# letao1991/EAD-GAN

Measured on AMD Instinct MI355X. Metric: imgs/sec per G+D+E train step, CelebA 64x64 bs=128, higher is better.
Workload: dtype bf16; 1 GPU; EAD-GAN CelebA 64x64x3 full train iteration (G adv + D + info/affine, 3 Adams), batch 128/GPU, hipGraph replay, data-parallel x1; per_gpu_batch=128, global_batch=128, parallelism=dp1

## Files before the change

ead-gan_amd/csrc/igemm_tn8.hip:

```cpp
#include <string.h>
#include <algorithm>

#include "eg_common.h"
#include "igemm_nt.h"

__device__ __forceinline__ int tn8_fsw(int row) { return (row & 3) | (((row >> 3) & 1) << 2); }

__device__ __forceinline__ void tn8_wait(int n) {
    switch (n) {
        case 0: __builtin_amdgcn_s_waitcnt(0 | (7 << 4)); break;
        case 1: __builtin_amdgcn_s_waitcnt(1 | (7 << 4)); break;
        case 2: __builtin_amdgcn_s_waitcnt(2 | (7 << 4)); break;
        case 3: __builtin_amdgcn_s_waitcnt(3 | (7 << 4)); break;
        case 4: __builtin_amdgcn_s_waitcnt(4 | (7 << 4)); break;
        case 5: __builtin_amdgcn_s_waitcnt(5 | (7 << 4)); break;
        case 6: __builtin_amdgcn_s_waitcnt(6 | (7 << 4)); break;
        default: __builtin_amdgcn_s_waitcnt(7 | (7 << 4)); break;
    }
}

template <typename T, int CH>
__global__ __launch_bounds__(512) void igemm_tn8_kernel(const Tn8Params p) {
    constexpr int ROWB = CH * 2;
    constexpr int RPP = 1024 / ROWB;
    constexpr int CPR = ROWB / 16;
    constexpr int NBLK = ROWB / 32;
    constexpr int NI = CH / 32, NJ = CH / 16;
    constexpr int NPP_P = (64 / RPP + 7) / 8;
    constexpr int PW_P = 64 / RPP < 8 ? 64 / RPP : 8;
    constexpr int STAGE_P = 64 * ROWB, STAGE_X = EG_TN8_XSLOTS * ROWB, STAGE = STAGE_P + STAGE_X;
    extern __shared__ __attribute__((aligned(16))) char smem[];
    const int tid = threadIdx.x, lane = tid & 63;
    const int wave = __builtin_amdgcn_readfirstlane(tid >> 6);
    const int tp = wave >> 1, nh = wave & 1;
    const int ay = tp >> 1, ax = tp & 1;
    const int tn_i = blockIdx.x / p.ntc, tc_i = blockIdx.x - tn_i * p.ntc;
    const int n0 = tn_i * CH, c0 = tc_i * CH;
    const int ry = blockIdx.y >> 1, rx = blockIdx.y & 1;
    const int mbeg = blockIdx.z * p.rows_per_split;
    const int mend = min(p.M, mbeg + p.rows_per_split);
    const int nk = (mend - mbeg) >> 6;
    const int OWm = (1 << p.lOW) - 1, OHm = (1 << p.lOH) - 1;
    const unsigned row_bytes = (unsigned)p.C * 2u;
    const int g = lane >> 4, li = lane & 15, q = li >> 2, pc = li & 3;

    int prow[4], xrow[4];
#pragma unroll
    for (int i = 0; i < 4; ++i) {
        const int r = (i >> 1) * 32 + 8 * g + (i & 1) * 4 + q;
        prow[i] = r * ROWB + (tn8_fsw(r) & (NBLK - 1));
        int img, oy;
        if (p.nimg == 1) { img = 0; oy = r >> p.lOW; }
        else { img = r >> (p.lOH + p.lOW); oy = (r >> p.lOW) & OHm; }
        const int px = (img * p.PH + oy + ay) * p.PW + (r & OWm) + ax;
        xrow[i] = px * ROWB + (tn8_fsw(px) & (NBLK - 1));
    }
    auto frag_addr = [&](int rowkey, int blk) { return (rowkey & ~7) + (((blk ^ (rowkey & 7)) << 5) | (pc << 3)); };

    const int c16 = lane % CPR, rsub = lane / CPR;
    const u32x4_t srdP = eg_make_srd(p.P, (unsigned)((size_t)p.M * p.N * 2));
    const u32x4_t srdX = eg_make_srd(p.src, (unsigned)((size_t)p.B * p.H * p.W * p.C * 2));
    unsigned vP[NPP_P];
#pragma unroll
    for (int j = 0; j < NPP_P; ++j) {
        const int r = RPP * (wave + 8 * j) + rsub;
        const int src16 = (((c16 >> 1) ^ (tn8_fsw(r) & (NBLK - 1))) << 1) | (c16 & 1);
        vP[j] = (unsigned)r * (unsigned)p.N * 2u + (unsigned)n0 * 2u + (unsigned)src16 * 16u;
    }
    int xa[5], xdy[5];
#pragma unroll
    for (int j = 0; j < 5; ++j) {
        const unsigned ps = (unsigned)(RPP * (wave + 8 * j) + rsub);
        const unsigned img = (ps * p.inv_plane) >> 20;
        const unsigned rem = ps - img * (unsigned)(p.PH * p.PW);
        const unsigned qy = (rem * p.inv_pw) >> 20, qx = rem - qy * (unsigned)p.PW;
        const int ix = (int)qx * 2 + rx - 1;
        const int src16 = (((c16 >> 1) ^ (tn8_fsw((int)ps) & (NBLK - 1))) << 1) | (c16 & 1);
        const bool ok = (int)ps < p.npix && ix >= 0 && ix < p.W;
        xdy[j] = (int)qy * 2 + ry - 1;
        xa[j] = ok ? (int)(((img * (unsigned)(p.H * p.W) + (unsigned)ix) * row_bytes) + (unsigned)c0 * 2u + (unsigned)src16 * 16u) : -1;
    }
    const unsigned lds0 = (unsigned)(size_t)(__attribute__((address_space(3))) char*)smem + (unsigned)wave * 1024u;

    auto issue = [&](int s, int stage) {
        const int m0s = mbeg + (s << 6);
        const unsigned base = __builtin_amdgcn_readfirstlane(lds0 + (unsigned)stage * STAGE);
        const unsigned soffP = (unsigned)m0s * (unsigned)p.N * 2u;
        if (PW_P == 8 || wave < PW_P) eg_bufdma1f<0>(srdP, vP[0], soffP, base);
        if constexpr (NPP_P > 1) eg_bufdma1f<0x2000>(srdP, vP[NPP_P - 1], soffP, base);
        const int b_s = m0s >> (p.lOH + p.lOW);
        const int oy_s = p.nimg == 1 ? ((m0s >> p.lOW) & OHm) : 0;
        const int ybase = oy_s * 2;
        const int pixbase = (b_s * p.H + ybase) * p.W;
#pragma unroll
        for (int j = 0; j < 5; ++j) {
            if (j < p.npp && (wave + 8 * j) * RPP < p.npix) {
                const int iy = ybase + xdy[j];
                const bool ok = xa[j] >= 0 && iy >= 0 && iy < p.H;
                const unsigned v = ok ? (unsigned)(xa[j] + (pixbase + xdy[j] * p.W) * (int)row_bytes) : EG_OOB;
                if (j == 0) eg_bufdma1f<STAGE_P>(srdX, v, 0u, base);
                if (j == 1) eg_bufdma1f<STAGE_P + 0x2000>(srdX, v, 0u, base);
                if (j == 2) eg_bufdma1f<STAGE_P + 0x4000>(srdX, v, 0u, base);
                if (j == 3) eg_bufdma1f<STAGE_P + 0x6000>(srdX, v, 0u, base);
                if (j == 4) eg_bufdma1f<STAGE_P + 0x8000>(srdX, v, 0u, base);
            }
        }
    };

    f32x4 acc[NI][NJ];
#pragma unroll
    for (int i = 0; i < NI; ++i)
#pragma unroll
        for (int j = 0; j < NJ; ++j) acc[i][j] = (f32x4){0.f, 0.f, 0.f, 0.f};

    typedef __attribute__((address_space(3))) s16x4* lds_s16x4;
    auto tr2 = [&](const char* base, int a_lo, int a_hi) {
        const s16x4 lo = __builtin_amdgcn_ds_read_tr16_b64_v4i16((lds_s16x4)(base + a_lo));
        const s16x4 hi = __builtin_amdgcn_ds_read_tr16_b64_v4i16((lds_s16x4)(base + a_hi));
        return make_uint4(((uint32_t)(uint16_t)lo[0]) | ((uint32_t)(uint16_t)lo[1] << 16), ((uint32_t)(uint16_t)lo[2]) | ((uint32_t)(uint16_t)lo[3] << 16),
                          ((uint32_t)(uint16_t)hi[0]) | ((uint32_t)(uint16_t)hi[1] << 16), ((uint32_t)(uint16_t)hi[2]) | ((uint32_t)(uint16_t)hi[3] << 16));
    };
    auto compute = [&](int stage) {
        const char* sp = smem + stage * STAGE;
        const char* sx = sp + STAGE_P;
#pragma unroll
        for (int kb = 0; kb < 2; ++kb) {
            uint4 af[NI], bfr[NJ];
#pragma unroll
            for (int i = 0; i < NI; ++i) af[i] = tr2(sp, frag_addr(prow[2 * kb], nh * NI + i), frag_addr(prow[2 * kb + 1], nh * NI + i));
#pragma unroll
            for (int j = 0; j < NJ; ++j) bfr[j] = tr2(sx, frag_addr(xrow[2 * kb], j), frag_addr(xrow[2 * kb + 1], j));
#pragma unroll
            for (int i = 0; i < NI; ++i)
#pragma unroll
                for (int j = 0; j < NJ; ++j) {
                    if constexpr (std::is_same<T, f16_t>::value)
                        acc[i][j] = __builtin_amdgcn_mfma_f32_16x16x32_f16(__builtin_bit_cast(f16x8_t, af[i]), __builtin_bit_cast(f16x8_t, bfr[j]), acc[i][j], 0, 0, 0);
                    else
                        acc[i][j] = __builtin_amdgcn_mfma_f32_16x16x32_bf16(__builtin_bit_cast(bf16x8_t, af[i]), __builtin_bit_cast(bf16x8_t, bfr[j]), acc[i][j], 0, 0, 0);
                }
        }
    };
    auto barrier = [&]() {
        __builtin_amdgcn_s_barrier();
        __builtin_amdgcn_sched_barrier(0);
    };

    int per = (PW_P == 8 || wave < PW_P) ? NPP_P : 0;
    for (int j = 0; j < p.npp; ++j) per += (wave + 8 * j) * RPP < p.npix;
    if (nk > 0) issue(0, 0);
    if (nk > 1) issue(1, 1);
    tn8_wait(nk > 1 ? per : 0);
    barrier();
    int st = 0;
    for (int t = 0; t < nk; ++t) {
        const int st2 = st == 0 ? 2 : st - 1;
        const bool more = t + 2 < nk;
        if (more) issue(t + 2, st2);
        compute(st);
        tn8_wait(more ? per : 0);
        barrier();
        st = st == 2 ? 0 : st + 1;
    }

    const int tap = (ry + 2 * ay) * 4 + (rx + 2 * ax);
    float* slab = p.slab + (size_t)blockIdx.z * p.N * 16 * p.C;
#pragma unroll
    for (int i = 0; i < NI; ++i)
#pragma unroll
        for (int r = 0; r < 4; ++r) {
            const int n = n0 + (nh * NI + i) * 16 + g * 4 + r;
            float* row = slab + ((size_t)n * 16 + tap) * p.C + c0 + li;
#pragma unroll
            for (int j = 0; j < NJ; ++j) row[j * 16] = acc[i][j][r];
        }
}

bool eg_tn8_plan(const eg_conv* c, int dtype, Tn8Params& p, int* nsplit, int wgs_target) {
    if (dtype == EG_F32 || c->k != 4 || c->stride != 2 || c->pad != 1 || c->up != 0) return false;
    const int ch = ((c->Cin % 128) == 0 && (c->Cout % 128) == 0) ? 128 : (((c->Cin % 64) == 0 && (c->Cout % 64) == 0) ? 64
                   : (((c->Cin % 32) == 0 && (c->Cout % 32) == 0) ? 32 : 0));
    if (ch == 0 || (c->H & 1) || (c->W & 1)) return false;
    const int OH = c->H / 2, OW = c->W / 2;
    const int lOH = ilog2_exact(OH), lOW = ilog2_exact(OW);
    const long long M = (long long)c->B * OH * OW;
    if (lOH < 0 || lOW < 0 || OW > 64 || (M % 64) != 0) return false;
    if ((size_t)c->B * c->H * c->W * c->Cin * 2 >= 0x7fffffffull || (size_t)M * c->Cout * 2 >= 0x7fffffffull) return false;
    memset(&p, 0, sizeof(p));
    p.B = c->B; p.H = c->H; p.W = c->W; p.C = c->Cin; p.N = c->Cout;
    p.lOH = lOH; p.lOW = lOW; p.M = (int)M;
    if (OH * OW >= 64) { p.nimg = 1; p.OHt = 64 / OW; }
    else { p.nimg = 64 / (OH * OW); p.OHt = OH; }
    p.PH = p.OHt + 1; p.PW = OW + 1;
    p.npix = p.nimg * p.PH * p.PW;
    p.ch = ch;
    const int rpp = 1024 / (ch * 2);
    if ((p.npix + rpp - 1) / rpp * rpp > EG_TN8_XSLOTS) return false;
    p.npp = ((p.npix + rpp - 1) / rpp + 7) / 8;
    if (p.npp > 5) return false;
    p.inv_pw = (1u << 20) / (unsigned)p.PW + 1;
    p.inv_plane = (1u << 20) / (unsigned)(p.PH * p.PW) + 1;
    for (unsigned x = 0; x < 512; ++x)
        if (((x * p.inv_pw) >> 20) != x / (unsigned)p.PW || ((x * p.inv_plane) >> 20) != x / (unsigned)(p.PH * p.PW)) return false;
    p.ntn = c->Cout / ch; p.ntc = c->Cin / ch;
    const long long base = (long long)p.ntn * p.ntc * 4;
    const int target = wgs_target > 0 ? wgs_target : 256;
    long long want = base >= target ? 1 : (target + base - 1) / base;
    const long long steps = M / 64;
    want = std::min(want, std::max(1LL, steps / 4));
    const long long sps = (steps + want - 1) / want;
    p.rows_per_split = (int)(sps * 64);
    *nsplit = (int)((steps + sps - 1) / sps);
    return true;
}

template <typename T, int CH>
static void launch_tn8_ch(const Tn8Params& p, int nsplit, hipStream_t st) {
    constexpr size_t lds = 3 * (size_t)(64 + EG_TN8_XSLOTS) * CH * 2;
    static bool attr_set = false;
    if (!attr_set) {
        (void)hipFuncSetAttribute(reinterpret_cast<const void*>(&igemm_tn8_kernel<T, CH>), hipFuncAttributeMaxDynamicSharedMemorySize, (int)lds);
        attr_set = true;
    }
    hipLaunchKernelGGL((igemm_tn8_kernel<T, CH>), dim3(p.ntn * p.ntc, 4, nsplit), dim3(512), lds, st, p);
}

template <typename T>
void eg_launch_tn8(const Tn8Params& p, int nsplit, hipStream_t st) {
    if (p.ch == 32) launch_tn8_ch<T, 32>(p, nsplit, st);
    else if (p.ch == 64) launch_tn8_ch<T, 64>(p, nsplit, st);
    else launch_tn8_ch<T, 128>(p, nsplit, st);
}
template void eg_launch_tn8<bf16_t>(const Tn8Params&, int, hipStream_t);
template void eg_launch_tn8<f16_t>(const Tn8Params&, int, hipStream_t);
```

Measured before the change: 30750 imgs/s.

## Software-pipeline LDS fragment reads with MFMA and interleave DMA issue in tn8 igemm

Restructures the main loop of the stride-2 4x4 weight-gradient implicit GEMM so fragments for the next k-half are read from LDS while MFMAs run on the current ones. DMA issue for stage t+3 is split into pieces spread across the MFMA loop, with one barrier per iteration placed between the halves. The prologue fills all three stages, and precomputed swizzled LDS addresses replace the per-access frag_addr math. It also simplifies the out-of-bounds checks and adds static asserts, at the cost of higher register pressure and fragile hand-placed waitcnt and barrier ordering.

New measurement: 31320 imgs/s, median of 6. 1.02x the previous value.

```diff
diff --git a/ead-gan_amd/csrc/igemm_tn8.hip b/ead-gan_amd/csrc/igemm_tn8.hip
--- a/ead-gan_amd/csrc/igemm_tn8.hip
+++ b/ead-gan_amd/csrc/igemm_tn8.hip
@@ -18,6 +18,18 @@
         default: __builtin_amdgcn_s_waitcnt(7 | (7 << 4)); break;
     }
 }
+__device__ __forceinline__ void tn8_wait2(int n) {
+    switch (n) {
+        case 2: __builtin_amdgcn_s_waitcnt(2 | (7 << 4)); break;
+        case 4: __builtin_amdgcn_s_waitcnt(4 | (7 << 4)); break;
+        case 6: __builtin_amdgcn_s_waitcnt(6 | (7 << 4)); break;
+        case 8: __builtin_amdgcn_s_waitcnt(8 | (7 << 4)); break;
+        case 10: __builtin_amdgcn_s_waitcnt(10 | (7 << 4)); break;
+        case 12: __builtin_amdgcn_s_waitcnt(12 | (7 << 4)); break;
+        case 14: __builtin_amdgcn_s_waitcnt(14 | (7 << 4)); break;
+        default: __builtin_amdgcn_s_waitcnt(0 | (7 << 4)); break;
+    }
+}
 
 template <typename T, int CH>
 __global__ __launch_bounds__(512) void igemm_tn8_kernel(const Tn8Params p) {
@@ -28,8 +40,12 @@
     constexpr int NI = CH / 32, NJ = CH / 16;
     constexpr int NPP_P = (64 / RPP + 7) / 8;
     constexpr int PW_P = 64 / RPP < 8 ? 64 / RPP : 8;
+    constexpr int NPP_X = (EG_TN8_XSLOTS / RPP + 7) / 8;
+    constexpr int PPG = (NPP_P + NPP_X + NJ - 1) / NJ;
     constexpr int STAGE_P = 64 * ROWB, STAGE_X = EG_TN8_XSLOTS * ROWB, STAGE = STAGE_P + STAGE_X;
-    extern __shared__ __attribute__((aligned(16))) char smem[];
+    static_assert(STAGE % ROWB == 0 && STAGE_P % ROWB == 0, "stage offsets keep the block bits of a row address clear");
+    static_assert(NPP_X <= 5 && NPP_P <= 2 && 2 * (NPP_P + NPP_X) <= 14, "piece tables, vmcnt range of tn8_wait");
+    extern __shared__ __attribute__((aligned(256))) char smem[];
     const int tid = threadIdx.x, lane = tid & 63;
     const int wave = __builtin_amdgcn_readfirstlane(tid >> 6);
     const int tp = wave >> 1, nh = wave & 1;
@@ -44,18 +60,21 @@
     const unsigned row_bytes = (unsigned)p.C * 2u;
     const int g = lane >> 4, li = lane & 15, q = li >> 2, pc = li & 3;
 
-    int prow[4], xrow[4];
+    int pk[NI], xk[4];
+    {
+        const int r = 8 * g + q, key = tn8_fsw(r) & (NBLK - 1);
+#pragma unroll
+        for (int i = 0; i < NI; ++i) pk[i] = r * ROWB + ((((nh * NI + i) ^ key) << 5) | (pc << 3));
+    }
 #pragma unroll
     for (int i = 0; i < 4; ++i) {
         const int r = (i >> 1) * 32 + 8 * g + (i & 1) * 4 + q;
-        prow[i] = r * ROWB + (tn8_fsw(r) & (NBLK - 1));
         int img, oy;
         if (p.nimg == 1) { img = 0; oy = r >> p.lOW; }
         else { img = r >> (p.lOH + p.lOW); oy = (r >> p.lOW) & OHm; }
         const int px = (img * p.PH + oy + ay) * p.PW + (r & OWm) + ax;
-        xrow[i] = px * ROWB + (tn8_fsw(px) & (NBLK - 1));
-    }
-    auto frag_addr = [&](int rowkey, int blk) { return (rowkey & ~7) + (((blk ^ (rowkey & 7)) << 5) | (pc << 3)); };
+        xk[i] = STAGE_P + px * ROWB + (((tn8_fsw(px) & (NBLK - 1)) << 5) | (pc << 3));
+    }
 
     const int c16 = lane % CPR, rsub = lane / CPR;
     const u32x4_t srdP = eg_make_srd(p.P, (unsigned)((size_t)p.M * p.N * 2));
@@ -67,9 +86,9 @@
         const int src16 = (((c16 >> 1) ^ (tn8_fsw(r) & (NBLK - 1))) << 1) | (c16 & 1);
         vP[j] = (unsigned)r * (unsigned)p.N * 2u + (unsigned)n0 * 2u + (unsigned)src16 * 16u;
     }
-    int xa[5], xdy[5];
-#pragma unroll
-    for (int j = 0; j < 5; ++j) {
+    int xa[NPP_X], xdy[NPP_X];
+#pragma unroll
+    for (int j = 0; j < NPP_X; ++j) {
         const unsigned ps = (unsigned)(RPP * (wave + 8 * j) + rsub);
         const unsigned img = (ps * p.inv_plane) >> 20;
         const unsigned rem = ps - img * (unsigned)(p.PH * p.PW);
@@ -77,32 +96,44 @@
         const int ix = (int)qx * 2 + rx - 1;
         const int src16 = (((c16 >> 1) ^ (tn8_fsw((int)ps) & (NBLK - 1))) << 1) | (c16 & 1);
         const bool ok = (int)ps < p.npix && ix >= 0 && ix < p.W;
-        xdy[j] = (int)qy * 2 + ry - 1;
-        xa[j] = ok ? (int)(((img * (unsigned)(p.H * p.W) + (unsigned)ix) * row_bytes) + (unsigned)c0 * 2u + (unsigned)src16 * 16u) : -1;
-    }
-    const unsigned lds0 = (unsigned)(size_t)(__attribute__((address_space(3))) char*)smem + (unsigned)wave * 1024u;
-
-    auto issue = [&](int s, int stage) {
+        const int dy = (int)qy * 2 + ry - 1;
+        xdy[j] = ok ? dy : 0x40000000;
+        xa[j] = (int)(((img * (unsigned)(p.H * p.W) + (unsigned)ix) * row_bytes) + (unsigned)c0 * 2u + (unsigned)src16 * 16u) + dy * p.W * (int)row_bytes;
+    }
+    const unsigned sm0 = (unsigned)(size_t)(__attribute__((address_space(3))) char*)smem;
+    const unsigned lds0 = sm0 + (unsigned)wave * 1024u;
+    const bool p_wave = PW_P == 8 || wave < PW_P;
+    int nxp = 0;
+    for (int j = 0; j < p.npp; ++j) nxp += (wave + 8 * j) * RPP < p.npix;
+    const int per = (p_wave ? NPP_P : 0) + nxp;
+
+    struct Step { unsigned base, soffP; int ybase, pixoff; };
+    auto step_of = [&](int s, int stage) {
+        Step d;
         const int m0s = mbeg + (s << 6);
-        const unsigned base = __builtin_amdgcn_readfirstlane(lds0 + (unsigned)stage * STAGE);
-        const unsigned soffP = (unsigned)m0s * (unsigned)p.N * 2u;
-        if (PW_P == 8 || wave < PW_P) eg_bufdma1f<0>(srdP, vP[0], soffP, base);
-        if constexpr (NPP_P > 1) eg_bufdma1f<0x2000>(srdP, vP[NPP_P - 1], soffP, base);
+        d.base = __builtin_amdgcn_readfirstlane(lds0 + (unsigned)stage * STAGE);
+        d.soffP = (unsigned)m0s * (unsigned)p.N * 2u;
         const int b_s = m0s >> (p.lOH + p.lOW);
-        const int oy_s = p.nimg == 1 ? ((m0s >> p.lOW) & OHm) : 0;
-        const int ybase = oy_s * 2;
-        const int pixbase = (b_s * p.H + ybase) * p.W;
-#pragma unroll
-        for (int j = 0; j < 5; ++j) {
-            if (j < p.npp && (wave + 8 * j) * RPP < p.npix) {
-                const int iy = ybase + xdy[j];
-                const bool ok = xa[j] >= 0 && iy >= 0 && iy < p.H;
-                const unsigned v = ok ? (unsigned)(xa[j] + (pixbase + xdy[j] * p.W) * (int)row_bytes) : EG_OOB;
-                if (j == 0) eg_bufdma1f<STAGE_P>(srdX, v, 0u, base);
-                if (j == 1) eg_bufdma1f<STAGE_P + 0x2000>(srdX, v, 0u, base);
-                if (j == 2) eg_bufdma1f<STAGE_P + 0x4000>(srdX, v, 0u, base);
-                if (j == 3) eg_bufdma1f<STAGE_P + 0x6000>(srdX, v, 0u, base);
-                if (j == 4) eg_bufdma1f<STAGE_P + 0x8000>(srdX, v, 0u, base);
+        d.ybase = p.nimg == 1 ? ((m0s >> p.lOW) & OHm) * 2 : 0;
+        d.pixoff = (b_s * p.H + d.ybase) * p.W * (int)row_bytes;
+        return d;
+    };
+    auto issue_piece = [&](const Step& d, int k) {
+        if (k < NPP_P) {
+            if (p_wave) {
+                if (k == 0) eg_bufdma1f<0>(srdP, vP[0], d.soffP, d.base);
+                if (k == 1) eg_bufdma1f<0x2000>(srdP, vP[NPP_P - 1], d.soffP, d.base);
+            }
+        } else if (k - NPP_P < NPP_X) {
+            const int j = k - NPP_P;
+            if (j < nxp) {
+                const int jj = j < NPP_X ? j : 0;
+                const unsigned v = (unsigned)(d.ybase + xdy[jj]) < (unsigned)p.H ? (unsigned)(xa[jj] + d.pixoff) : EG_OOB;
+                if (j == 0) eg_bufdma1f<STAGE_P>(srdX, v, 0u, d.base);
+                if (j == 1) eg_bufdma1f<STAGE_P + 0x2000>(srdX, v, 0u, d.base);
+                if (j == 2) eg_bufdma1f<STAGE_P + 0x4000>(srdX, v, 0u, d.base);
+                if (j == 3) eg_bufdma1f<STAGE_P + 0x6000>(srdX, v, 0u, d.base);
+                if (j == 4) eg_bufdma1f<STAGE_P + 0x8000>(srdX, v, 0u, d.base);
             }
         }
     };
@@ -114,53 +145,74 @@
         for (int j = 0; j < NJ; ++j) acc[i][j] = (f32x4){0.f, 0.f, 0.f, 0.f};
 
     typedef __attribute__((address_space(3))) s16x4* lds_s16x4;
-    auto tr2 = [&](const char* base, int a_lo, int a_hi) {
-        const s16x4 lo = __builtin_amdgcn_ds_read_tr16_b64_v4i16((lds_s16x4)(base + a_lo));
-        const s16x4 hi = __builtin_amdgcn_ds_read_tr16_b64_v4i16((lds_s16x4)(base + a_hi));
+    auto tr2 = [&](unsigned a_lo, unsigned a_hi) {
+        const s16x4 lo = __builtin_amdgcn_ds_read_tr16_b64_v4i16((lds_s16x4)(size_t)a_lo);
+        const s16x4 hi = __builtin_amdgcn_ds_read_tr16_b64_v4i16((lds_s16x4)(size_t)a_hi);
         return make_uint4(((uint32_t)(uint16_t)lo[0]) | ((uint32_t)(uint16_t)lo[1] << 16), ((uint32_t)(uint16_t)lo[2]) | ((uint32_t)(uint16_t)lo[3] << 16),
                           ((uint32_t)(uint16_t)hi[0]) | ((uint32_t)(uint16_t)hi[1] << 16), ((uint32_t)(uint16_t)hi[2]) | ((uint32_t)(uint16_t)hi[3] << 16));
     };
-    auto compute = [&](int stage) {
-        const char* sp = smem + stage * STAGE;
-        const char* sx = sp + STAGE_P;
-#pragma unroll
-        for (int kb = 0; kb < 2; ++kb) {
-            uint4 af[NI], bfr[NJ];
-#pragma unroll
-            for (int i = 0; i < NI; ++i) af[i] = tr2(sp, frag_addr(prow[2 * kb], nh * NI + i), frag_addr(prow[2 * kb + 1], nh * NI + i));
-#pragma unroll
-            for (int j = 0; j < NJ; ++j) bfr[j] = tr2(sx, frag_addr(xrow[2 * kb], j), frag_addr(xrow[2 * kb + 1], j));
-#pragma unroll
-            for (int i = 0; i < NI; ++i)
-#pragma unroll
-                for (int j = 0; j < NJ; ++j) {
-                    if constexpr (std::is_same<T, f16_t>::value)
-                        acc[i][j] = __builtin_amdgcn_mfma_f32_16x16x32_f16(__builtin_bit_cast(f16x8_t, af[i]), __builtin_bit_cast(f16x8_t, bfr[j]), acc[i][j], 0, 0, 0);
-                    else
-                        acc[i][j] = __builtin_amdgcn_mfma_f32_16x16x32_bf16(__builtin_bit_cast(bf16x8_t, af[i]), __builtin_bit_cast(bf16x8_t, bfr[j]), acc[i][j], 0, 0, 0);
+    uint4 af0[NI], af1[NI], bfr[NJ];
+    auto publish = [&](int n, auto widec) {
+        asm volatile("" ::: "memory");
+        __builtin_amdgcn_sched_barrier(0);
+        if (decltype(widec)::value) tn8_wait2(n);
+        else tn8_wait(n);
+        __builtin_amdgcn_s_barrier();
+        asm volatile("" ::: "memory");
+        __builtin_amdgcn_sched_barrier(0);
+    };
+    auto half = [&](const uint4 (&ca)[NI], uint4 (&na)[NI], int soff, auto kbc, auto dmc, const Step& d, bool dm) {
+        constexpr int kb = decltype(kbc)::value;
+        constexpr bool DM = decltype(dmc)::value;
+        const unsigned sb = sm0 + (unsigned)soff, sp = sb + kb * 32 * ROWB;
+        const unsigned x_lo = sb + (unsigned)xk[2 * kb], x_hi = sb + (unsigned)xk[2 * kb + 1];
+#pragma unroll
+        for (int j = 0; j < NJ; ++j) {
+#pragma unroll
+            for (int i = 0; i < NI; ++i) {
+                if constexpr (std::is_same<T, f16_t>::value)
+                    acc[i][j] = __builtin_amdgcn_mfma_f32_16x16x32_f16(__builtin_bit_cast(f16x8_t, ca[i]), __builtin_bit_cast(f16x8_t, bfr[j]), acc[i][j], 0, 0, 0);
+                else
+                    acc[i][j] = __builtin_amdgcn_mfma_f32_16x16x32_bf16(__builtin_bit_cast(bf16x8_t, ca[i]), __builtin_bit_cast(bf16x8_t, bfr[j]), acc[i][j], 0, 0, 0);
+            }
+            bfr[j] = tr2(x_lo ^ (unsigned)(j << 5), x_hi ^ (unsigned)(j << 5));
+            if (j < NI) na[j] = tr2(sp + (unsigned)pk[j], sp + (unsigned)pk[j] + 4 * ROWB);
+            if constexpr (DM) {
+                if (dm) {
+#pragma unroll
+                    for (int k = j * PPG; k < (j + 1) * PPG; ++k) issue_piece(d, k);
                 }
+            }
+            __builtin_amdgcn_sched_barrier(0);
         }
     };
-    auto barrier = [&]() {
-        __builtin_amdgcn_s_barrier();
-        __builtin_amdgcn_sched_barrier(0);
-    };
-
-    int per = (PW_P == 8 || wave < PW_P) ? NPP_P : 0;
-    for (int j = 0; j < p.npp; ++j) per += (wave + 8 * j) * RPP < p.npix;
-    if (nk > 0) issue(0, 0);
-    if (nk > 1) issue(1, 1);
-    tn8_wait(nk > 1 ? per : 0);
-    barrier();
+
+    const int npro = min(nk, 3);
+    for (int s = 0; s < npro; ++s) {
+        const Step d = step_of(s, s);
+#pragma unroll
+        for (int k = 0; k < NPP_P + NPP_X; ++k) issue_piece(d, k);
+    }
+    publish(per * max(npro - 1, 0), std::true_type{});
+    {
+        const unsigned x_lo = sm0 + (unsigned)xk[0], x_hi = sm0 + (unsigned)xk[1];
+#pragma unroll
+        for (int j = 0; j < NJ; ++j) bfr[j] = tr2(x_lo ^ (unsigned)(j << 5), x_hi ^ (unsigned)(j << 5));
+#pragma unroll
+        for (int i = 0; i < NI; ++i) af0[i] = tr2(sm0 + (unsigned)pk[i], sm0 + (unsigned)pk[i] + 4 * ROWB);
+    }
+    asm volatile("" ::: "memory");
+    __builtin_amdgcn_s_waitcnt(0xc07f);
+    __builtin_amdgcn_sched_barrier(0);
     int st = 0;
     for (int t = 0; t < nk; ++t) {
-        const int st2 = st == 0 ? 2 : st - 1;
-        const bool more = t + 2 < nk;
-        if (more) issue(t + 2, st2);
-        compute(st);
-        tn8_wait(more ? per : 0);
-        barrier();
-        st = st == 2 ? 0 : st + 1;
+        const int st1 = st == 2 ? 0 : st + 1;
+        const bool dm = t + 3 < nk;
+        const Step d = step_of(t + 3, st);
+        half(af0, af1, st * STAGE, std::integral_constant<int, 1>{}, std::false_type{}, d, false);
+        publish(t + 2 < nk ? per : 0, std::false_type{});
+        half(af1, af0, st1 * STAGE, std::integral_constant<int, 0>{}, std::true_type{}, d, dm);
+        st = st1;
     }
 
     const int tap = (ry + 2 * ay) * 4 + (rx + 2 * ax);
```
